# netneurolab/pypyls

Hardware: AMD Instinct MI355X
Metric: resamples/sec (perm+boot), behavioral_pls X(500x200000)/Y(500x50) fp64 (higher is better)
Workload: dtype f64

## Files before the change

pypyls_amd/csrc/plsx_compact.hip:

```cpp
#include "plsx_internal.h"

using namespace plsxi;

namespace plsxi {

template <int MT, int KT, bool TAIL = false>
int launch_xprod_cboot(plsx_ctx* ctx, int nres, int nks_c, SplitEpi se, hipStream_t st)
{
    const size_t stage = (size_t)2 * (((size_t)KT * MT * 64 + 127) / 128) * 128 * 8 + (size_t)nks_c * 4 * sizeof(int);
    const size_t epi = (size_t)se.npairs * 128 * 8 + (size_t)2 * MT * 16 * 4;
    const size_t lds = std::max(stage, epi);
    HIPCHK(set_lds(k_xprod_compact<MT, KT, 3, TAIL>, lds));
    const int ncolblk = ceil_div(ctx->Bpad, 128);
    KTimer tm(ctx, KC_XPROD, st);
    hipLaunchKernelGGL((k_xprod_compact<MT, KT, 3, TAIL>), dim3(round_up(ncolblk, 8) * round_up(nres, 8)), dim3(256),
                       lds, st, ptr<double>(ctx->Afrag_c), (size_t)nks_c * MT * 64, ptr<double>(ctx->Xc), ctx->Bpad, nks_c,
                       ptr<double>(ctx->R), ctx->Bpad, ctx->Tpp, ptr<int>(ctx->out_row_c), ptr<int>(ctx->mom_idx_c),
                       (const double*)nullptr, nres, ncolblk, se);
    LAUNCHCHK();
    return 0;
}

int launch_cboot(plsx_ctx* ctx, int nres, int nks_c, SplitEpi se, hipStream_t st)
{
    const int MTc = ceil_div(ctx->Tp, 16);
    const bool tail = ctx->Tp - (MTc - 1) * 16 <= 4 && MTc >= 2;
    switch (MTc) {
        case 1: return launch_xprod_cboot<1, 12>(ctx, nres, nks_c, se, st);
        case 2: return tail ? launch_xprod_cboot<2, 6, true>(ctx, nres, nks_c, se, st)
                            : launch_xprod_cboot<2, 6>(ctx, nres, nks_c, se, st);
        case 3: return tail ? launch_xprod_cboot<3, 4, true>(ctx, nres, nks_c, se, st)
                            : launch_xprod_cboot<3, 4>(ctx, nres, nks_c, se, st);
        case 4: return tail ? launch_xprod_cboot<4, PLSX_CKT, true>(ctx, nres, nks_c, se, st)
                            : launch_xprod_cboot<4, PLSX_CKT>(ctx, nres, nks_c, se, st);
#define PLSX_CB(M, K) case M: return tail ? launch_xprod_cboot<M, K, true>(ctx, nres, nks_c, se, st) \
                                          : launch_xprod_cboot<M, K>(ctx, nres, nks_c, se, st);
        PLSX_CB(5, 2) PLSX_CB(6, 2) PLSX_CB(7, 1) PLSX_CB(8, 1) PLSX_CB(9, 1) PLSX_CB(10, 1) PLSX_CB(11, 1) PLSX_CB(12, 1) PLSX_CB(13, 1)
#undef PLSX_CB
        default: return fail(ctx, PLSX_ERR_STATE, "compact bootstrap blocks: T' > 208");
    }
}
template <int MT, int KT, bool TAIL = false, int EPI = 5>
int launch_xprod_compact(plsx_ctx* ctx, int m, int nks_c, SplitEpi se, hipStream_t st)
{
    const int J = ctx->J;
    const size_t stage = (size_t)2 * (((size_t)KT * MT * 64 + 127) / 128) * 128 * 8 + (size_t)nks_c * 4 * sizeof(int);
    const size_t epi = EPI == 8 ? (size_t)MT * 16 * 4 : (size_t)5 * J * 128 * 8 + (size_t)2 * MT * 16 * 4 + (size_t)MT * 16 * 5 * 8;
    const size_t lds = std::max(stage, epi);
    se.off_pre = 0;
    HIPCHK(set_lds(k_xprod_compact<MT, KT, EPI, TAIL>, lds));
    const int ncolblk = ceil_div(ctx->Bpad, 128);
    KTimer tm(ctx, KC_XPROD, st);
    hipLaunchKernelGGL((k_xprod_compact<MT, KT, EPI, TAIL>), dim3(round_up(ncolblk, 8) * round_up(m, 8)), dim3(256), lds, st,
                       ptr<double>(ctx->Afrag_c), (size_t)nks_c * MT * 64, ptr<double>(ctx->Xc), ctx->Bpad, nks_c,
                       ptr<double>(ctx->R), ctx->Bpad, (EPI == 8 ? 1 : 2) * ctx->Tpp, ptr<int>(ctx->out_row_c), ptr<int>(ctx->mom_idx_c),
                       ptr<double>(ctx->momn_m), m, ncolblk, se);
    LAUNCHCHK();
    return 0;
}

int launch_csplit(plsx_ctx* ctx, int m, int nks_c, SplitEpi se, hipStream_t st, bool raw)
{
    const int MTc = ceil_div(ctx->Tp, 16);
    const bool tail = ctx->Tp - (MTc - 1) * 16 <= 4;
    if (raw) {
        switch (MTc) {
            case 2: return tail ? launch_xprod_compact<2, 6, true, 8>(ctx, m, nks_c, se, st)
                                : launch_xprod_compact<2, 6, false, 8>(ctx, m, nks_c, se, st);
            case 3: return tail ? launch_xprod_compact<3, 4, true, 8>(ctx, m, nks_c, se, st)
                                : launch_xprod_compact<3, 4, false, 8>(ctx, m, nks_c, se, st);
            case 4: if (tail) return launch_xprod_compact<4, PLSX_CKT, true, 8>(ctx, m, nks_c, se, st);
                    [[fallthrough]];
            default: return fail(ctx, PLSX_ERR_STATE, "raw compact split blocks: T' outside 17..52");
        }
    }
    switch (MTc) {
        case 1: return launch_xprod_compact<1, 12>(ctx, m, nks_c, se, st);
        case 2: return tail ? launch_xprod_compact<2, 6, true>(ctx, m, nks_c, se, st)
                            : launch_xprod_compact<2, 6>(ctx, m, nks_c, se, st);
        case 3: return tail ? launch_xprod_compact<3, 4, true>(ctx, m, nks_c, se, st)
                            : launch_xprod_compact<3, 4>(ctx, m, nks_c, se, st);
        default: return tail ? launch_xprod_compact<4, PLSX_CKT, true>(ctx, m, nks_c, se, st)
                             : launch_xprod_compact<4, PLSX_CKT>(ctx, m, nks_c, se, st);
    }
}

}
```

pypyls_amd/csrc/plsx_k_xprod.h:

```cpp
#pragma once
#include <type_traits>
#include <utility>

template <class F, int... I>
__device__ __forceinline__ void xprod_static_for(F&& f, std::integer_sequence<int, I...>)
{
    (f(std::integral_constant<int, I>()), ...);
}
#include "plsx_common.h"
#include "plsx_k_prep.h"

#define PLSX_RSRC_FLAGS 0x00020000
template <int NT, int PASSES, bool EVEN, int STAGE>
__device__ __forceinline__ void stage_copy_buf(const double* src, double* dst, int tid, int wave)
{
    __amdgpu_buffer_rsrc_t rs = __builtin_amdgcn_make_buffer_rsrc((void*)src, (short)0, 0x7fffffff,
                                                                   PLSX_RSRC_FLAGS);
    const int voff = tid * 16;
#pragma unroll
    for (int p = 0; p < PASSES; ++p) {
        if (EVEN || p * NT + wave * 64 < STAGE / 2) {
            __builtin_amdgcn_raw_ptr_buffer_load_lds(
                rs, (__attribute__((address_space(3))) void*)(dst + (size_t)(p * NT + wave * 64) * 2),
                16, voff, p * NT * 16, 0, 0);
        }
    }
}

__device__ __forceinline__ double load_x_buf(const double* rowbase, int voff)
{
    __amdgpu_buffer_rsrc_t rs = __builtin_amdgcn_make_buffer_rsrc((void*)rowbase, (short)0, 0x7fffffff,
                                                                   PLSX_RSRC_FLAGS);
    return __builtin_bit_cast(double, __builtin_amdgcn_raw_buffer_load_b64(rs, voff, 0, 0));
}

#define PLSX_ACC_PITCH 80
template <int MT, int NW, int KT, int NSQ, int EPI = 0>
__global__ __launch_bounds__(NW * 64, 2)
void k_xprod(const double* __restrict__ Afrag, size_t group_stride,
             const double* __restrict__ X, int ldx, int nks,
             double* __restrict__ R, int ldr, int rows_per_group,
             const int* __restrict__ out_row, const int* __restrict__ mom_idx,
             const double* __restrict__ mom_n, int nmom_pad,
             int n_groups, int ncolblk, double* __restrict__ mom_out, SplitEpi se, int ntab)
{
    extern __shared__ __attribute__((aligned(16))) double smem[];
    constexpr int NT = NW * 64;
    constexpr int STAGE = KT * MT * 64;
    constexpr int STAGE_LDS = ((STAGE + 127) / 128) * 128;
    constexpr int PASSES = (STAGE + NT * 2 - 1) / (NT * 2);
    constexpr bool EVEN = (STAGE % (NT * 2)) == 0;
    const int tid = threadIdx.x;
    const int lane = tid & 63, wave = tid >> 6;
    const int sweep = blockIdx.x / (8 * ncolblk);
    const int within = blockIdx.x - sweep * (8 * ncolblk);
    int grp = sweep * 8 + (within & 7);
    int colblk = within >> 3;
    if (sweep * 8 + 8 > n_groups) {
        const int rem = n_groups - sweep * 8;
        const int cnt = (rem * ncolblk + 7) >> 3;
        const int id = (within & 7) * cnt + colblk;
        if (colblk >= cnt || id >= rem * ncolblk) return;
        grp = sweep * 8 + id / ncolblk;
        colblk = id - (id / ncolblk) * ncolblk;
    }
    const int col = colblk * (NW * 16) + wave * 16 + (lane & 15);
    const int kq = lane >> 4;

    static_assert(EPI != 7 || KT == 1 || KT == 2 || KT == 4, "EPI 7: the four k-steps of a tile row are whole stages");
    const int qblk = (EPI == 7) ? grp / max(se.J, 1) : 0;
    const int ks0 = (EPI == 7) ? qblk * (MT * 4) : 0;
    if (EPI == 7) { X += (size_t)ks0 * 4 * ldx; nks -= ks0; }
    const double* Ag = Afrag + (size_t)grp * group_stride + (size_t)ks0 * (MT * 64);
    const int swave = __builtin_amdgcn_readfirstlane(wave);
    const int xvoff = (kq * ldx + min(col, ldx - 1)) * 8;

    d4 acc[MT];
#pragma unroll
    for (int m = 0; m < MT; ++m) acc[m] = (d4){0.0, 0.0, 0.0, 0.0};

    const int nkt = nks / KT;
    constexpr bool SPLIT = (EPI == 1);
    if constexpr (SPLIT) {
        if (se.off_pre > 0 && NW == 4) {
            double* sRf = smem + se.off_pre;
            double* sRc = sRf + se.Tpp * (NW * 16);
            __amdgpu_buffer_rsrc_t rsF = __builtin_amdgcn_make_buffer_rsrc(
                (void*)(se.Rfull + (size_t)colblk * (NW * 16)), (short)0, 0x7fffffff, PLSX_RSRC_FLAGS);
            const int vo = ((lane >> 5) * ldr + (lane & 31) * 2) * 8;
            for (int j = swave; j < se.Tpp / 2; j += NW)
                __builtin_amdgcn_raw_ptr_buffer_load_lds(
                    rsF, (__attribute__((address_space(3))) void*)(sRf + j * 128), 16, vo, j * 2 * ldr * 8, 0, 0);
            __amdgpu_buffer_rsrc_t rsC = __builtin_amdgcn_make_buffer_rsrc(
                (void*)(se.rowc + (size_t)grp * MT * 16 * 5), (short)0, 0x7fffffff, PLSX_RSRC_FLAGS);
            for (int pc = swave; pc < (MT * 16 * 5 + 127) / 128; pc += NW)
                __builtin_amdgcn_raw_ptr_buffer_load_lds(
                    rsC, (__attribute__((address_space(3))) void*)(sRc + pc * 128), 16, lane * 16, pc * 1024, 0, 0);
        }
    }
    stage_copy_buf<NT, PASSES, EVEN, STAGE>(Ag, smem, tid, swave);
    double xb[KT];
#pragma unroll
    for (int s = 0; s < KT; ++s)
        xb[s] = load_x_buf(X + (size_t)(s * 4) * ldx, xvoff);
#pragma unroll
    for (int s = 0; s < KT; ++s) asm volatile("" : "+v"(xb[s]));
    __syncthreads();

    auto pass = [&](int kt, auto na) {
        constexpr int NA = decltype(na)::value;
        const int cur = kt & 1;
        const int kn = min(kt + 1, nkt - 1);
        double xn[KT];
        stage_copy_buf<NT, PASSES, EVEN, STAGE>(Ag + (size_t)kn * STAGE, smem + (cur ^ 1) * STAGE_LDS, tid, swave);
#pragma unroll
        for (int s = 0; s < KT; ++s)
            xn[s] = load_x_buf(X + (size_t)((kn * KT + s) * 4) * ldx, xvoff);
        const double* sA = smem + cur * STAGE_LDS + lane;
#pragma unroll
        for (int s = 0; s < KT; ++s) {
            const double b = xb[s];
            const double bsq = (NSQ > 0) ? b * b : 0.0;
#pragma unroll
            for (int m = 0; m < NA; ++m)
                acc[m] = mfma_f64(sA[(s * MT + m) * 64], (m < MT - NSQ) ? b : bsq, acc[m]);
        }
#pragma unroll
        for (int s = 0; s < KT; ++s) xb[s] = xn[s];
        __syncthreads();
    };
    int kt_first = 0;
    if constexpr (EPI == 7) {
        xprod_static_for([&](auto mm) {
#pragma unroll
            for (int j = 0; j < 4 / KT; ++j) {
                const int kt = (4 / KT) * decltype(mm)::value + j;
                if (kt < nkt) pass(kt, std::integral_constant<int, decltype(mm)::value + 1>());
            }
        }, std::make_integer_sequence<int, MT>());
        kt_first = min(nkt, 4 * MT / KT);
    }
    for (int kt = kt_first; kt < nkt; ++kt) pass(kt, std::integral_constant<int, MT>());

    constexpr int W0 = MT - 2 * NSQ, SQ0 = MT - NSQ, NMOM = NSQ * 16;
    if constexpr (EPI == 6) {
        static_assert(MT == 2 * NSQ, "EPI 6 is a moment-only instantiation");
#pragma unroll
        for (int j = 0; j < NSQ; ++j)
#pragma unroll
            for (int i = 0; i < 4; ++i) {
                const int pair = grp * (NSQ * 16) + j * 16 + kq + 4 * i;
                if (pair >= se.npairs || col >= ldr) continue;
                se.scale[(size_t)pair * ldr + col] = acc[j][i];
                se.scale2[(size_t)pair * ldr + col] = acc[NSQ + j][i];
            }
        return;
    }
    if constexpr (EPI == 4) {
        static_assert(MT == 2 * NSQ, "EPI 4 is the moment-only instantiation");
#pragma unroll
        for (int j = 0; j < NSQ; ++j)
#pragma unroll
            for (int i = 0; i < 4; ++i) {
                const int pair = grp * (NSQ * 16) + j * 16 + kq + 4 * i;
                if (pair >= se.npairs || col >= ldr) continue;
                const double m1 = acc[j][i], m2 = acc[NSQ + j][i];
                const double nn = mom_n[pair];
                const double var = (m2 - m1 * m1 / nn) / (nn - 1.0);
                se.scale[(size_t)pair * ldr + col] = (var > 0.0) ? sd_rsqrt(var) : 0.0;
            }
        return;
    }
    if constexpr (EPI == 3) {
        const int nmu = se.npairs;
        double* sS3 = smem;
        int* s_out = reinterpret_cast<int*>(smem + (size_t)nmu * (NW * 16));
        int* s_mom = s_out + MT * 16;
        const double* sc0 = se.scale + (size_t)grp * nmu * ldr + colblk * (NW * 16);
        for (int idx = tid; idx < nmu * (NW * 16); idx += NT) {
            const int mi = idx / (NW * 16), c = idx - mi * (NW * 16);
            sS3[idx] = sc0[(size_t)mi * ldr + c];
        }
        for (int i = tid; i < MT * 16; i += NT) { s_out[i] = out_row[i]; s_mom[i] = mom_idx[i]; }
        __syncthreads();
        double* Rg = R + (size_t)grp * rows_per_group * ldr + col;
        const int cw = wave * 16 + (lane & 15);
        const int rows_valid = min(rows_per_group, se.accB - grp * rows_per_group);
#pragma unroll
        for (int m = 0; m < MT; ++m) {
            int orow[4];
            double sc[4];
#pragma unroll
            for (int i = 0; i < 4; ++i) {
                const int row = m * 16 + kq + 4 * i;
                orow[i] = s_out[row];
                const int mi = s_mom[row];
                sc[i] = mi >= 0 ? sS3[mi * (NW * 16) + cw] : 1.0;
            }
#pragma unroll
            for (int i = 0; i < 4; ++i)
                if (orow[i] >= 0 && orow[i] < rows_valid) Rg[(size_t)orow[i] * ldr] = acc[m][i] * sc[i];
        }
        return;
    }
    if constexpr (EPI == 7) {
        if (NW > 4 && col >= ldr) return;
        const int s0 = qblk * (MT * 16);
        const int Srows = se.accB;
        const double* Xc = X + col - (size_t)(ks0 * 4) * ldx;
        double part = 0.0;
#pragma unroll
        for (int m = 0; m < MT; ++m) {
            double xv[4];
#pragma unroll
            for (int i = 0; i < 4; ++i) {
                const int sr = s0 + m * 16 + kq + 4 * i;
                const double x = Xc[(size_t)min(sr, Srows - 1) * ldx];
                xv[i] = sr < Srows ? x : 0.0;
            }
#pragma unroll
            for (int i = 0; i < 4; ++i) part = __builtin_fma(xv[i], acc[m][i], part);
            asm volatile("" : "+v"(part));
        }
        part += __shfl_xor(part, 16);
        part += __shfl_xor(part, 32);
        if (kq == 0) se.acc_sum[(size_t)grp * ldr + col] = part;
        return;
    }
    if constexpr (EPI == 2) {
        constexpr int ACCP = NW * 16 + 16;
        constexpr int BCW = NW * 16;
        const int L = se.accL;
        double* sU = smem;
        double* sV = smem + (size_t)L * ACCP;
        double* sT = sV + (size_t)L * ACCP;
        int* s_l = reinterpret_cast<int*>(sT + 32 * ACCP);
        for (int i = tid; i < 2 * L * ACCP; i += NT) smem[i] = 0.0;
        for (int i = tid; i < MT * 16; i += NT) s_l[i] = out_row[i];
        const int cw = wave * 16 + (lane & 15);
#pragma unroll
        for (int m0 = 0; m0 < MT; m0 += 2) {
            __syncthreads();
#pragma unroll
            for (int mm = 0; mm < 2; ++mm)
#pragma unroll
                for (int i = 0; i < 4; ++i)
                    if (m0 + mm < MT) sT[(mm * 16 + kq + 4 * i) * ACCP + cw] = acc[m0 + mm][i];
            __syncthreads();
            for (int idx = tid; idx < L * BCW; idx += NT) {
                const int l = idx / BCW, c = idx - l * BCW;
                double u = sU[l * ACCP + c], v2 = sV[l * ACCP + c];
                for (int rl = 0; rl < 32 && m0 * 16 + rl < MT * 16; ++rl)
                    if (s_l[m0 * 16 + rl] == l) { const double v = sT[rl * ACCP + c]; u += v; v2 += v * v; }
                sU[l * ACCP + c] = u; sV[l * ACCP + c] = v2;
            }
        }
        __syncthreads();
        const int b0 = colblk * (NW * 16);
        double* ps = se.acc_sum + (size_t)grp * se.accB * L;
        double* pq = se.acc_sq + (size_t)grp * se.accB * L;
        for (int idx = tid; idx < NW * 16 * L; idx += NT) {
            const int c = idx / L, l = idx - c * L;
            if (b0 + c < se.accB) {
                ps[(size_t)(b0 + c) * L + l] = sU[l * ACCP + c];
                pq[(size_t)(b0 + c) * L + l] = sV[l * ACCP + c];
            }
        }
        return;
    }
    if constexpr (SPLIT && NSQ > 0) {
        const int nmu = se.nmu;
        const bool pre = se.off_pre > 0 && NW == 4;
        double* w5 = smem + wave * (5 * nmu * 16);
        int* s_out = reinterpret_cast<int*>(smem + NW * 5 * nmu * 16);
        int* s_mom = s_out + MT * 16;
        const double* sRf = smem + se.off_pre;
        double* s_rc = pre ? smem + se.off_pre + se.Tpp * (NW * 16)
                           : reinterpret_cast<double*>(s_mom + MT * 16);
        const int pitch2 = 2 * se.Tpp;
        for (int i = tid; i < MT * 16; i += NT) {
            const int orw = out_row[i];
            s_out[i] = orw < 0 ? -1 : (orw | ((orw % pitch2) << 20));
            s_mom[i] = mom_idx[i];
        }
        if (!pre)
            for (int i = tid; i < MT * 16 * 5; i += NT) s_rc[i] = se.rowc[(size_t)grp * MT * 16 * 5 + i];
#pragma unroll
        for (int j = 0; j < NSQ; ++j)
#pragma unroll
            for (int i = 0; i < 4; ++i) {
                const int mr = j * 16 + kq + 4 * i;
                if (mr >= nmu) continue;
                const int o = mr * 16 + (lane & 15);
                const double n1 = mom_n[(size_t)grp * nmom_pad + mr];
                const double m1 = acc[W0 + j][i], m2 = acc[SQ0 + j][i];
                const int jc = mr % se.J;
                const double nF = (double)se.cell_len[jc];
                const double SF = se.cellS1[(size_t)jc * ldr + col], SFF = se.cellS2[(size_t)jc * ldr + col];
                const double n2 = nF - n1;
                const bool ok = n1 > 1.5 && n2 > 1.5;
                const double var1 = ok ? (m2 - m1 * m1 / n1) / (n1 - 1.0) : 0.0;
                const double s2x = SF - m1, s2xx = SFF - m2;
                const double var2 = ok ? (s2xx - s2x * s2x / n2) / (n2 - 1.0) : 0.0;
                const double varF = (SFF - SF * SF / nF) / (nF - 1.0);
                w5[0 * nmu * 16 + o] = ok ? m1 / n1 : 0.0;
                w5[1 * nmu * 16 + o] = (var1 > 0.0) ? 1.0 / sqrt(var1) : 0.0;
                w5[2 * nmu * 16 + o] = ok ? s2x / n2 : 0.0;
                w5[3 * nmu * 16 + o] = (var2 > 0.0) ? 1.0 / sqrt(var2) : 0.0;
                w5[4 * nmu * 16 + o] = (varF > 0.0) ? sqrt(varF) : 0.0;
            }
        __syncthreads();
        double* Rg = R + (size_t)grp * rows_per_group * ldr + col;
#pragma unroll
        for (int m = 0; m < W0; ++m)
#pragma unroll
            for (int i = 0; i < 4; ++i) {
                const int row = m * 16 + kq + 4 * i;
                const int packed = s_out[row];
                if (packed < 0) continue;
                const int orow = packed & 0xfffff, t = packed >> 20;
                const int o = s_mom[row] * 16 + (lane & 15);
                const double* rc = s_rc + row * 5;
                const double c1 = acc[m][i];
                const double rf = pre ? sRf[t * (NW * 16) + wave * 16 + (lane & 15)]
                                      : se.Rfull[(size_t)t * ldr + col];
                const double cf = rf * rc[4] * w5[4 * nmu * 16 + o];
                const double r1 = (c1 - rc[0] * w5[o]) * rc[1] * w5[1 * nmu * 16 + o];
                const double r2 = ((cf - c1) - rc[2] * w5[2 * nmu * 16 + o]) * rc[3] * w5[3 * nmu * 16 + o];
                __builtin_nontemporal_store(r1, &Rg[(size_t)orow * ldr]);
                __builtin_nontemporal_store(r2, &Rg[(size_t)(orow + se.Tpp) * ldr]);
            }
        return;
    }
    double* sS = smem + wave * (2 * NMOM * 16);
    double* sQ = sS + NMOM * 16;
    int* s_out = reinterpret_cast<int*>(smem + NW * 2 * NMOM * 16);
    int* s_mom = s_out + MT * 16;
    const int tab = (ntab > 1) ? (grp % ntab) * (MT * 16) : 0;
    for (int i = tid; i < MT * 16; i += NT) { s_out[i] = out_row[tab + i]; s_mom[i] = mom_idx[tab + i]; }
    if (NSQ > 0) {
#pragma unroll
        for (int j = 0; j < NSQ; ++j)
#pragma unroll
            for (int i = 0; i < 4; ++i) {
                sS[j * 256 + (kq + 4 * i) * 16 + (lane & 15)] = acc[W0 + j][i];
                sQ[j * 256 + (kq + 4 * i) * 16 + (lane & 15)] = acc[SQ0 + j][i];
            }
    }
    __syncthreads();
    if (NSQ > 0) {
        for (int mr = kq; mr < NMOM; mr += 4) {
            const int o = mr * 16 + (lane & 15);
            const double m1 = sS[o], m2 = sQ[o];
            const double nn = mom_n[(size_t)grp * nmom_pad + mr];
            const double var = (m2 - m1 * m1 / nn) / (nn - 1.0);
            const double sc = (var > 0.0) ? 1.0 / sqrt(var) : 0.0;
            sS[o] = sc;
            if (mom_out) {
                double* mo = mom_out + ((size_t)grp * nmom_pad + mr) * 2 * ldr + col;
                mo[0] = m1 / nn;
                mo[ldr] = sc;
            }
        }
        __syncthreads();
    }
    if (NW > 4 && col >= ldr) return;
    double* Rg = R + (size_t)(ntab > 1 ? grp / ntab : grp) * rows_per_group * ldr + col;
#pragma unroll
    for (int m = 0; m < W0; ++m) {
        int orow[4];
        double sc[4];
#pragma unroll
        for (int i = 0; i < 4; ++i) {
            const int row = m * 16 + kq + 4 * i;
            orow[i] = s_out[row];
            const int mi = s_mom[row];
            sc[i] = (NSQ > 0 && mi >= 0) ? sS[mi * 16 + (lane & 15)] : 1.0;
        }
#pragma unroll
        for (int i = 0; i < 4; ++i)
            if (orow[i] >= 0) Rg[(size_t)orow[i] * ldr] = acc[m][i] * sc[i];
    }
}

__device__ __forceinline__ d2 load_x2_buf(const double* base, int voff)
{
    __amdgpu_buffer_rsrc_t rs = __builtin_amdgcn_make_buffer_rsrc((void*)base, (short)0, 0x7fffffff, PLSX_RSRC_FLAGS);
    return __builtin_bit_cast(d2, __builtin_amdgcn_raw_buffer_load_b128(rs, voff, 0, 0));
}

template <int MT, int KT, int EPI, bool TAIL>
__global__ __launch_bounds__(256, MT > 6 ? 2 : ((MT > 4 || (EPI == 5 && MT == 4 && !TAIL)) ? 3 : 4))
void k_xprod_compact(const double* __restrict__ Afrag, size_t group_stride,
                     const double* __restrict__ X, int ldx, int nks,
                     double* __restrict__ R, int ldr, int rows_per_group,
                     const int* __restrict__ out_row, const int* __restrict__ mom_idx,
                     const double* __restrict__ mom_n, int n_groups, int ncolblk, SplitEpi se)
{
    static_assert(EPI == 3 || EPI == 5 || EPI == 8, "compact blocks: bootstrap (3), fused split-half (5) or raw first-half sums (8)");
    extern __shared__ __attribute__((aligned(16))) double smem[];
    constexpr int NW = 4, NT = NW * 64, BC = NW * 32;
    constexpr int STAGE = KT * MT * 64;
    constexpr int STAGE_LDS = ((STAGE + 127) / 128) * 128;
    constexpr int PASSES = (STAGE + NT * 2 - 1) / (NT * 2);
    constexpr bool EVEN = (STAGE % (NT * 2)) == 0;
    constexpr int MF = TAIL ? MT - 1 : MT;
    const int tid = threadIdx.x, lane = tid & 63, wave = tid >> 6;
    const int ncb = (ncolblk + 7) & ~7;
    const int sweep = blockIdx.x / (8 * ncb);
    const int within = blockIdx.x - sweep * (8 * ncb);
    const int slot = within >> 3;
    const int grp = sweep * 8 + (slot & 7);
    const int colblk = (slot >> 3) * 8 + (within & 7);
    if (grp >= n_groups || colblk >= ncolblk) return;
    const int kq = lane >> 4;
    const int cw = wave * 32 + 2 * (lane & 15);
    const int col = colblk * BC + cw;
    const bool live = col < ldr;
    const int lcol = live ? col : 0;
    const double* Ag = Afrag + (size_t)grp * group_stride;
    const int swave = __builtin_amdgcn_readfirstlane(wave);

    d4 acc0[MF > 0 ? MF : 1], acc1[MF > 0 ? MF : 1];
#pragma unroll
    for (int m = 0; m < MF; ++m) { acc0[m] = (d4){0.0, 0.0, 0.0, 0.0}; acc1[m] = (d4){0.0, 0.0, 0.0, 0.0}; }
    double tl0 = 0.0, tl1 = 0.0;
    const int toff = (lane & 48) + (lane & 3) - lane;

    const int ksteps = max(1, (se.row_cnt[grp] + 3) >> 2);
    const int nkt = (ksteps + KT - 1) / KT;
    int* s_tab = reinterpret_cast<int*>(smem + 2 * STAGE_LDS);
    for (int i = tid; i < nks * 4; i += NT) s_tab[i] = se.row_tab[(size_t)grp * nks * 4 + i];
    __syncthreads();
    auto x_off = [&](int kstep) -> int { return (s_tab[kstep * 4 + kq] * ldx + lcol) * 8; };

    stage_copy_buf<NT, PASSES, EVEN, STAGE>(Ag, smem, tid, swave);
    d2 xb[KT];
#pragma unroll
    for (int s = 0; s < KT; ++s) xb[s] = load_x2_buf(X, x_off(s));
#pragma unroll
    for (int s = 0; s < KT; ++s) asm volatile("" : "+v"(xb[s]));
    __syncthreads();

    auto pass = [&](int kt, auto full) {
        const int cur = kt & 1;
        const int kn = min(kt + 1, nkt - 1);
        d2 xn[KT];
        stage_copy_buf<NT, PASSES, EVEN, STAGE>(Ag + (size_t)kn * STAGE, smem + (cur ^ 1) * STAGE_LDS, tid, swave);
#pragma unroll
        for (int s = 0; s < KT; ++s) xn[s] = load_x2_buf(X, x_off(kn * KT + s));
        const double* sA = smem + cur * STAGE_LDS + lane;
#pragma unroll
        for (int s = 0; s < KT; ++s) {
            if constexpr (!decltype(full)::value) {
                if (kt * KT + s >= ksteps) break;
            }
            const double b0 = xb[s].x, b1 = xb[s].y;
#pragma unroll
            for (int m = 0; m < MF; ++m) {
                const double a = sA[(s * MT + m) * 64];
                acc0[m] = mfma_f64(a, b0, acc0[m]);
                acc1[m] = mfma_f64(a, b1, acc1[m]);
            }
            if constexpr (TAIL) {
                const double a = sA[(s * MT + MT - 1) * 64 + toff];
                tl0 = mfma_f64_4x4(a, b0, tl0);
                tl1 = mfma_f64_4x4(a, b1, tl1);
            }
        }
#pragma unroll
        for (int s = 0; s < KT; ++s) xb[s] = xn[s];
        __syncthreads();
    };
    const int nfull = ksteps / KT;
    int kt_main = 0;
    for (; kt_main < nfull; ++kt_main) pass(kt_main, std::integral_constant<bool, true>());
    for (; kt_main < nkt; ++kt_main) pass(kt_main, std::integral_constant<bool, false>());

    auto val0 = [&](int m, int i) -> double { return (TAIL && m == MT - 1) ? tl0 : acc0[m < MF ? m : 0][i]; };
    auto val1 = [&](int m, int i) -> double { return (TAIL && m == MT - 1) ? tl1 : acc1[m < MF ? m : 0][i]; };

    if constexpr (EPI == 8) {
        int* s_out = reinterpret_cast<int*>(smem);
        for (int i = tid; i < MT * 16; i += NT) s_out[i] = out_row[i];
        __syncthreads();
        if (!live) return;
        double* Rg = R + (size_t)grp * rows_per_group * ldr + col;
#pragma unroll
        for (int m = 0; m < MT; ++m)
#pragma unroll
            for (int i = 0; i < 4; ++i) {
                if (TAIL && m == MT - 1 && i > 0) break;
                const int orow = s_out[m * 16 + kq + 4 * i];
                if (orow < 0) continue;
                __builtin_nontemporal_store((d2){val0(m, i), val1(m, i)}, reinterpret_cast<d2*>(&Rg[(size_t)orow * ldr]));
            }
        return;
    } else if constexpr (EPI == 3) {
        const int nmu = se.npairs;
        double* sS3 = smem;
        int* s_out = reinterpret_cast<int*>(smem + (size_t)nmu * BC);
        int* s_mom = s_out + MT * 16;
        const double* sc0 = se.scale + (size_t)grp * nmu * ldr + colblk * BC;
        for (int idx = tid; idx < nmu * BC; idx += NT) {
            const int mi = idx / BC, c = idx - mi * BC;
            sS3[idx] = (colblk * BC + c < ldr) ? sc0[(size_t)mi * ldr + c] : 0.0;
        }
        for (int i = tid; i < MT * 16; i += NT) { s_out[i] = out_row[i]; s_mom[i] = mom_idx[i]; }
        __syncthreads();
        if (!live) return;
        double* Rg = R + (size_t)grp * rows_per_group * ldr + col;
        const int rows_valid = min(rows_per_group, se.accB - grp * rows_per_group);
#pragma unroll
        for (int m = 0; m < MT; ++m)
#pragma unroll
            for (int i = 0; i < 4; ++i) {
                if (TAIL && m == MT - 1 && i > 0) break;
                const int row = m * 16 + kq + 4 * i;
                const int orow = s_out[row], mi = s_mom[row];
                if (orow < 0 || orow >= rows_valid) continue;
                d2 sc = (d2){1.0, 1.0};
                if (mi >= 0) sc = *reinterpret_cast<const d2*>(&sS3[mi * BC + cw]);
                *reinterpret_cast<d2*>(&Rg[(size_t)orow * ldr]) = (d2){val0(m, i) * sc.x, val1(m, i) * sc.y};
            }
        return;
    } else {
        const int J = se.J;
        double* w5 = smem;
        int* s_out = reinterpret_cast<int*>(smem + (size_t)5 * J * BC);
        int* s_mom = s_out + MT * 16;
        double* s_rc = reinterpret_cast<double*>(s_mom + MT * 16);
        const int pitch2 = 2 * se.Tpp;
        for (int i = tid; i < MT * 16; i += NT) {
            const int orw = out_row[i];
            s_out[i] = orw < 0 ? -1 : (orw | ((orw % pitch2) << 20));
            s_mom[i] = mom_idx[i];
        }
        for (int i = tid; i < MT * 16 * 5; i += NT) s_rc[i] = se.rowc[(size_t)grp * MT * 16 * 5 + i];
        const int cb0 = colblk * BC;
        for (int idx = tid; idx < J * BC; idx += NT) {
            const int jc = idx / BC, c = idx - jc * BC;
            double u1 = 0, v1 = 0, u2 = 0, v2 = 0, sF = 0;
            if (cb0 + c < ldr) {
                const size_t pair = (size_t)grp * J + jc;
                const double n1 = mom_n[pair];
                const double m1 = se.scale[pair * ldr + cb0 + c], m2 = se.scale2[pair * ldr + cb0 + c];
                const double nF = (double)se.cell_len[jc];
                const double SF = se.cellS1[(size_t)jc * ldr + cb0 + c], SFF = se.cellS2[(size_t)jc * ldr + cb0 + c];
                const double n2 = nF - n1;
                const bool ok = n1 > 1.5 && n2 > 1.5;
                const double var1 = ok ? (m2 - m1 * m1 / n1) / (n1 - 1.0) : 0.0;
                const double s2x = SF - m1, s2xx = SFF - m2;
                const double var2 = ok ? (s2xx - s2x * s2x / n2) / (n2 - 1.0) : 0.0;
                const double varF = (SFF - SF * SF / nF) / (nF - 1.0);
                u1 = ok ? m1 / n1 : 0.0;
                v1 = (var1 > 0.0) ? 1.0 / sqrt(var1) : 0.0;
                u2 = ok ? s2x / n2 : 0.0;
                v2 = (var2 > 0.0) ? 1.0 / sqrt(var2) : 0.0;
                sF = (varF > 0.0) ? sqrt(varF) : 0.0;
            }
            const int o = jc * BC + c;
            w5[0 * J * BC + o] = u1; w5[1 * J * BC + o] = v1; w5[2 * J * BC + o] = u2;
            w5[3 * J * BC + o] = v2; w5[4 * J * BC + o] = sF;
        }
        __syncthreads();
        if (!live) return;
        double* Rg = R + (size_t)grp * rows_per_group * ldr + col;
        const int JW = J * BC;
#pragma unroll
        for (int m = 0; m < MT; ++m)
#pragma unroll
            for (int i = 0; i < 4; ++i) {
                if (TAIL && m == MT - 1 && i > 0) break;
                const int row = m * 16 + kq + 4 * i;
                const int packed = s_out[row];
                if (packed < 0) continue;
                const int o = s_mom[row] * BC + cw;
                const double rc0 = s_rc[row * 5], rc1 = s_rc[row * 5 + 1];
                const d2 u1 = *reinterpret_cast<const d2*>(&w5[o]), v1 = *reinterpret_cast<const d2*>(&w5[JW + o]);
                const d2 r1 = (d2){(val0(m, i) - rc0 * u1.x) * rc1 * v1.x, (val1(m, i) - rc0 * u1.y) * rc1 * v1.y};
                __builtin_nontemporal_store(r1, reinterpret_cast<d2*>(&Rg[(size_t)(packed & 0xfffff) * ldr]));
            }
#pragma unroll
        for (int m0 = 0; m0 < MT; m0 += 2) {
            asm volatile("" ::: "memory");
            d2 rfv[2][4];
#pragma unroll
            for (int mm = 0; mm < 2; ++mm)
#pragma unroll
                for (int i = 0; i < 4; ++i) {
                    const int m = m0 + mm;
                    if (m >= MT || (TAIL && m == MT - 1 && i > 0)) break;
                    const int packed = s_out[m * 16 + kq + 4 * i];
                    rfv[mm][i] = packed < 0 ? (d2){0.0, 0.0}
                                            : *reinterpret_cast<const d2*>(&se.Rfull[(size_t)(packed >> 20) * ldr + col]);
                }
#pragma unroll
            for (int mm = 0; mm < 2; ++mm)
#pragma unroll
                for (int i = 0; i < 4; ++i) {
                    const int m = m0 + mm;
                    if (m >= MT || (TAIL && m == MT - 1 && i > 0)) break;
                    const int row = m * 16 + kq + 4 * i;
                    const int packed = s_out[row];
                    if (packed < 0) continue;
                    const int o = s_mom[row] * BC + cw;
                    const double rc2 = s_rc[row * 5 + 2], rc3 = s_rc[row * 5 + 3], rc4 = s_rc[row * 5 + 4];
                    const d2 u2 = *reinterpret_cast<const d2*>(&w5[2 * JW + o]), v2 = *reinterpret_cast<const d2*>(&w5[3 * JW + o]);
                    const d2 sF = *reinterpret_cast<const d2*>(&w5[4 * JW + o]);
                    const double c10 = val0(m, i), c11 = val1(m, i);
                    const double cf0 = rfv[mm][i].x * rc4 * sF.x, cf1 = rfv[mm][i].y * rc4 * sF.y;
                    const d2 r2 = (d2){((cf0 - c10) - rc2 * u2.x) * rc3 * v2.x, ((cf1 - c11) - rc2 * u2.y) * rc3 * v2.y};
                    __builtin_nontemporal_store(r2, reinterpret_cast<d2*>(&Rg[(size_t)((packed & 0xfffff) + se.Tpp) * ldr]));
                }
        }
    }
}
```

Measured before the change: 5956.

## Restructure compact xprod kernel prologue, double-buffer ping-pong and epilogue row maps

Reworks the compact cross-product kernel so the row-map and row-table staging overlaps with the first X and A loads. The table is pre-scaled by ldx*8, and the k-loop is unrolled into a static two-buffer ping-pong with register swap. In the bootstrap epilogue the output-row and moment-index maps are packed into one int. Scale factors come from registers when few pairs exist, otherwise they are loaded async to per-wave LDS. LDS sizing is centralised and occupancy hints per MT are retuned. The aim is fewer syncthreads, less epilogue staging and more occupancy, at the cost of added complexity and register pressure.

Result: faster. 6023, median of 6 (+1.1%).

```diff
diff --git a/pypyls_amd/csrc/plsx_compact.hip b/pypyls_amd/csrc/plsx_compact.hip
--- a/pypyls_amd/csrc/plsx_compact.hip
+++ b/pypyls_amd/csrc/plsx_compact.hip
@@ -7,9 +7,7 @@
 template <int MT, int KT, bool TAIL = false>
 int launch_xprod_cboot(plsx_ctx* ctx, int nres, int nks_c, SplitEpi se, hipStream_t st)
 {
-    const size_t stage = (size_t)2 * (((size_t)KT * MT * 64 + 127) / 128) * 128 * 8 + (size_t)nks_c * 4 * sizeof(int);
-    const size_t epi = (size_t)se.npairs * 128 * 8 + (size_t)2 * MT * 16 * 4;
-    const size_t lds = std::max(stage, epi);
+    const size_t lds = compact_lds_bytes(MT, KT, 3, nks_c, se.npairs);
     HIPCHK(set_lds(k_xprod_compact<MT, KT, 3, TAIL>, lds));
     const int ncolblk = ceil_div(ctx->Bpad, 128);
     KTimer tm(ctx, KC_XPROD, st);
@@ -44,9 +42,7 @@
 int launch_xprod_compact(plsx_ctx* ctx, int m, int nks_c, SplitEpi se, hipStream_t st)
 {
     const int J = ctx->J;
-    const size_t stage = (size_t)2 * (((size_t)KT * MT * 64 + 127) / 128) * 128 * 8 + (size_t)nks_c * 4 * sizeof(int);
-    const size_t epi = EPI == 8 ? (size_t)MT * 16 * 4 : (size_t)5 * J * 128 * 8 + (size_t)2 * MT * 16 * 4 + (size_t)MT * 16 * 5 * 8;
-    const size_t lds = std::max(stage, epi);
+    const size_t lds = compact_lds_bytes(MT, KT, EPI, nks_c, J);
     se.off_pre = 0;
     HIPCHK(set_lds(k_xprod_compact<MT, KT, EPI, TAIL>, lds));
     const int ncolblk = ceil_div(ctx->Bpad, 128);
diff --git a/pypyls_amd/csrc/plsx_k_xprod.h b/pypyls_amd/csrc/plsx_k_xprod.h
--- a/pypyls_amd/csrc/plsx_k_xprod.h
+++ b/pypyls_amd/csrc/plsx_k_xprod.h
@@ -389,8 +389,24 @@
     return __builtin_bit_cast(d2, __builtin_amdgcn_raw_buffer_load_b128(rs, voff, 0, 0));
 }
 
+__host__ __device__ constexpr int compact_stage_lds(int MT, int KT) { return ((KT * MT * 64 + 127) / 128) * 128; }
+__host__ __device__ constexpr int compact_scale_regs(int KT) { return KT < 4 ? KT : 4; }
+__host__ __device__ constexpr size_t compact_lds_bytes(int MT, int KT, int EPI, int nks, int J)
+{
+    const size_t loop = (size_t)MT * 16 * 8 + (size_t)2 * compact_stage_lds(MT, KT) * 8 + (size_t)nks * 4 * 4;
+    if (EPI == 3) return loop + (J > compact_scale_regs(KT) ? (size_t)J * 128 * 8 : 0);
+    const size_t epi5 = (size_t)MT * 16 * 8 + (size_t)5 * J * 128 * 8 + (size_t)MT * 16 * 5 * 8;
+    return EPI == 5 && epi5 > loop ? epi5 : loop;
+}
+
+__host__ __device__ constexpr int compact_waves(int MT, int EPI, bool TAIL)
+{
+    if (EPI == 3) return MT > 10 ? 2 : MT == 10 ? (TAIL ? 3 : 2) : MT > 6 ? 3 : MT > 4 ? 4 : (MT == 4 && TAIL) ? 5 : 4;
+    return (EPI == 5 && MT == 4 && !TAIL) ? 3 : 4;
+}
+
 template <int MT, int KT, int EPI, bool TAIL>
-__global__ __launch_bounds__(256, MT > 6 ? 2 : ((MT > 4 || (EPI == 5 && MT == 4 && !TAIL)) ? 3 : 4))
+__global__ __launch_bounds__(256, compact_waves(MT, EPI, TAIL))
 void k_xprod_compact(const double* __restrict__ Afrag, size_t group_stride,
                      const double* __restrict__ X, int ldx, int nks,
                      double* __restrict__ R, int ldr, int rows_per_group,
@@ -401,11 +417,12 @@
     extern __shared__ __attribute__((aligned(16))) double smem[];
     constexpr int NW = 4, NT = NW * 64, BC = NW * 32;
     constexpr int STAGE = KT * MT * 64;
-    constexpr int STAGE_LDS = ((STAGE + 127) / 128) * 128;
+    constexpr int STAGE_LDS = compact_stage_lds(MT, KT);
     constexpr int PASSES = (STAGE + NT * 2 - 1) / (NT * 2);
     constexpr bool EVEN = (STAGE % (NT * 2)) == 0;
     constexpr int MF = TAIL ? MT - 1 : MT;
-    const int tid = threadIdx.x, lane = tid & 63, wave = tid >> 6;
+    constexpr int NSCR = compact_scale_regs(KT);
+    static_assert(MT * 16 <= NT, "the row maps are staged by one thread per row");
     const int ncb = (ncolblk + 7) & ~7;
     const int sweep = blockIdx.x / (8 * ncb);
     const int within = blockIdx.x - sweep * (8 * ncb);
@@ -413,49 +430,87 @@
     const int grp = sweep * 8 + (slot & 7);
     const int colblk = (slot >> 3) * 8 + (within & 7);
     if (grp >= n_groups || colblk >= ncolblk) return;
+    const double* Ag = Afrag + (size_t)grp * group_stride;
+    const int swave = __builtin_amdgcn_readfirstlane((int)threadIdx.x >> 6);
+
+    d4 acc0[MF > 0 ? MF : 1], acc1[MF > 0 ? MF : 1];
+#pragma unroll
+    for (int m = 0; m < MF; ++m) { acc0[m] = (d4){0.0, 0.0, 0.0, 0.0}; acc1[m] = (d4){0.0, 0.0, 0.0, 0.0}; }
+    double tl0 = 0.0, tl1 = 0.0;
+
+    int* s_out = reinterpret_cast<int*>(smem);
+    int* s_mom = s_out + MT * 16;
+    double* sStage = smem + MT * 16;
+    int* s_tab = reinterpret_cast<int*>(sStage + 2 * STAGE_LDS);
+    const int J3 = se.npairs;
+    double* sW = reinterpret_cast<double*>(s_tab + nks * 4) + swave * (J3 * 32);
+    d2 scr[NSCR];
+    {
+    const int tid = threadIdx.x, lane = tid & 63, wave = tid >> 6;
     const int kq = lane >> 4;
     const int cw = wave * 32 + 2 * (lane & 15);
     const int col = colblk * BC + cw;
     const bool live = col < ldr;
-    const int lcol = live ? col : 0;
-    const double* Ag = Afrag + (size_t)grp * group_stride;
-    const int swave = __builtin_amdgcn_readfirstlane(wave);
-
-    d4 acc0[MF > 0 ? MF : 1], acc1[MF > 0 ? MF : 1];
-#pragma unroll
-    for (int m = 0; m < MF; ++m) { acc0[m] = (d4){0.0, 0.0, 0.0, 0.0}; acc1[m] = (d4){0.0, 0.0, 0.0, 0.0}; }
-    double tl0 = 0.0, tl1 = 0.0;
+    const int lcol8 = (live ? col : 0) * 8;
     const int toff = (lane & 48) + (lane & 3) - lane;
 
+    const int* tabg = se.row_tab + (size_t)grp * nks * 4;
+    const int ldx8 = ldx * 8;
+    int row0[KT];
+#pragma unroll
+    for (int s = 0; s < KT; ++s) row0[s] = tabg[s * 4 + kq];
+    stage_copy_buf<NT, PASSES, EVEN, STAGE>(Ag, sStage, tid, swave);
+    int orw = -1, mix = -1;
+    if (tid < MT * 16) {
+        orw = out_row[tid];
+        if (EPI != 8) mix = mom_idx[tid];
+    }
     const int ksteps = max(1, (se.row_cnt[grp] + 3) >> 2);
     const int nkt = (ksteps + KT - 1) / KT;
-    int* s_tab = reinterpret_cast<int*>(smem + 2 * STAGE_LDS);
-    for (int i = tid; i < nks * 4; i += NT) s_tab[i] = se.row_tab[(size_t)grp * nks * 4 + i];
+    const int ntab = nkt * KT * 4;
+    auto tab_load = [&](int i0, int (&v)[4]) {
+#pragma unroll
+        for (int u = 0; u < 4; ++u) v[u] = tabg[min(i0 + u * NT + tid, ntab - 1)];
+#pragma unroll
+        for (int u = 0; u < 4; ++u) asm volatile("" : "+v"(v[u]));
+    };
+    auto tab_store = [&](int i0, const int (&v)[4]) {
+#pragma unroll
+        for (int u = 0; u < 4; ++u)
+            if (i0 + u * NT + tid < ntab) s_tab[i0 + u * NT + tid] = v[u] * ldx8;
+    };
+    int tv[4];
+    tab_load(0, tv);
+    d2 xa[KT], xb[KT];
+#pragma unroll
+    for (int s = 0; s < KT; ++s) xa[s] = load_x2_buf(X, row0[s] * ldx8 + lcol8);
+    tab_store(0, tv);
+    for (int i0 = 4 * NT; i0 < ntab; i0 += 4 * NT) { tab_load(i0, tv); tab_store(i0, tv); }
+    if (tid < MT * 16) {
+        if constexpr (EPI == 3) {
+            const int rows_valid = min(rows_per_group, se.accB - grp * rows_per_group);
+            s_out[tid] = (orw < 0 || orw >= rows_valid) ? -1 : (orw | ((mix + 1) << 16));
+        } else if constexpr (EPI == 5) {
+            s_out[tid] = orw < 0 ? -1 : (orw | ((orw % (2 * se.Tpp)) << 20));
+            s_mom[tid] = mix;
+        } else {
+            s_out[tid] = orw;
+        }
+    }
+#pragma unroll
+    for (int s = 0; s < KT; ++s) asm volatile("" : "+v"(xa[s]));
     __syncthreads();
-    auto x_off = [&](int kstep) -> int { return (s_tab[kstep * 4 + kq] * ldx + lcol) * 8; };
-
-    stage_copy_buf<NT, PASSES, EVEN, STAGE>(Ag, smem, tid, swave);
-    d2 xb[KT];
-#pragma unroll
-    for (int s = 0; s < KT; ++s) xb[s] = load_x2_buf(X, x_off(s));
-#pragma unroll
-    for (int s = 0; s < KT; ++s) asm volatile("" : "+v"(xb[s]));
-    __syncthreads();
-
-    auto pass = [&](int kt, auto full) {
-        const int cur = kt & 1;
-        const int kn = min(kt + 1, nkt - 1);
-        d2 xn[KT];
-        stage_copy_buf<NT, PASSES, EVEN, STAGE>(Ag + (size_t)kn * STAGE, smem + (cur ^ 1) * STAGE_LDS, tid, swave);
-#pragma unroll
-        for (int s = 0; s < KT; ++s) xn[s] = load_x2_buf(X, x_off(kn * KT + s));
-        const double* sA = smem + cur * STAGE_LDS + lane;
+
+    const double* sA0 = sStage + lane;
+    const double* sT0 = sA0 + toff;
+    auto contract = [&](auto curc, const d2 (&xc)[KT], auto full, int nlive) {
+        const int cur = curc;
+        const double* sA = sA0 + cur * STAGE_LDS;
+        const double* sT = sT0 + cur * STAGE_LDS;
 #pragma unroll
         for (int s = 0; s < KT; ++s) {
-            if constexpr (!decltype(full)::value) {
-                if (kt * KT + s >= ksteps) break;
-            }
-            const double b0 = xb[s].x, b1 = xb[s].y;
+            if (!decltype(full)::value && s >= nlive) continue;
+            const double b0 = xc[s].x, b1 = xc[s].y;
 #pragma unroll
             for (int m = 0; m < MF; ++m) {
                 const double a = sA[(s * MT + m) * 64];
@@ -463,27 +518,70 @@
                 acc1[m] = mfma_f64(a, b1, acc1[m]);
             }
             if constexpr (TAIL) {
-                const double a = sA[(s * MT + MT - 1) * 64 + toff];
+                const double a = sT[(s * MT + MT - 1) * 64];
                 tl0 = mfma_f64_4x4(a, b0, tl0);
                 tl1 = mfma_f64_4x4(a, b1, tl1);
             }
         }
-#pragma unroll
-        for (int s = 0; s < KT; ++s) xb[s] = xn[s];
+    };
+    const int* tp = s_tab + KT * 4 + kq;
+    const double* An = Ag + STAGE;
+    auto pass = [&](auto curc, const d2 (&xc)[KT], d2 (&xn)[KT]) {
+        constexpr int CUR = decltype(curc)::value;
+        stage_copy_buf<NT, PASSES, EVEN, STAGE>(An, sStage + (CUR ^ 1) * STAGE_LDS, tid, swave);
+#pragma unroll
+        for (int s = 0; s < KT; ++s) xn[s] = load_x2_buf(X, tp[s * 4] + lcol8);
+        An += STAGE;
+        tp += KT * 4;
+        contract(curc, xc, std::true_type(), KT);
         __syncthreads();
     };
-    const int nfull = ksteps / KT;
-    int kt_main = 0;
-    for (; kt_main < nfull; ++kt_main) pass(kt_main, std::integral_constant<bool, true>());
-    for (; kt_main < nkt; ++kt_main) pass(kt_main, std::integral_constant<bool, false>());
-
+    auto last = [&](int cur, const d2 (&xc)[KT]) {
+#pragma unroll
+        for (int j = 0; j < NSCR; ++j) scr[j] = (d2){1.0, 1.0};
+        if constexpr (EPI == 3) {
+            if (J3 <= NSCR) {
+#pragma unroll
+                for (int j = 0; j < NSCR; ++j)
+                    if (j < J3)
+                        scr[j] = *reinterpret_cast<const d2*>(
+                            reinterpret_cast<const char*>(se.scale + ((size_t)grp * J3 + j) * ldr) + lcol8);
+            } else if (live) {
+                __amdgpu_buffer_rsrc_t rs = __builtin_amdgcn_make_buffer_rsrc(
+                    (void*)(se.scale + (size_t)grp * J3 * ldr + colblk * BC + swave * 32), (short)0, 0x7fffffff, PLSX_RSRC_FLAGS);
+                const int ln4 = __lane_id() * 4;
+                for (int j = 0; j < J3; ++j)
+                    __builtin_amdgcn_raw_ptr_buffer_load_lds(
+                        rs, (__attribute__((address_space(3))) void*)(sW + j * 32), 4, ln4, j * ldr * 8, 0, 0);
+            }
+        }
+        contract(cur, xc, std::false_type(), ksteps - (nkt - 1) * KT);
+        if constexpr (EPI == 5) __syncthreads();
+    };
+    {
+        std::integral_constant<int, 0> c0;
+        std::integral_constant<int, 1> c1;
+        int kt = 0, cur = 0;
+        for (; kt + 2 < nkt; kt += 2) { pass(c0, xa, xb); pass(c1, xb, xa); }
+        if (kt + 1 < nkt) {
+            pass(c0, xa, xb);
+#pragma unroll
+            for (int s = 0; s < KT; ++s) xa[s] = xb[s];
+            cur = 1;
+        }
+        last(cur, xa);
+    }
+    }
+
+    int tid16 = threadIdx.x * 16;
+    if constexpr (EPI != 5) asm volatile("" : "+v"(tid16));
+    const int tid = tid16 >> 4, lane = tid & 63, wave = tid >> 6, kq = lane >> 4;
+    const int cw = wave * 32 + 2 * (lane & 15), col = colblk * BC + cw;
+    const bool live = col < ldr;
     auto val0 = [&](int m, int i) -> double { return (TAIL && m == MT - 1) ? tl0 : acc0[m < MF ? m : 0][i]; };
     auto val1 = [&](int m, int i) -> double { return (TAIL && m == MT - 1) ? tl1 : acc1[m < MF ? m : 0][i]; };
 
     if constexpr (EPI == 8) {
-        int* s_out = reinterpret_cast<int*>(smem);
-        for (int i = tid; i < MT * 16; i += NT) s_out[i] = out_row[i];
-        __syncthreads();
         if (!live) return;
         double* Rg = R + (size_t)grp * rows_per_group * ldr + col;
 #pragma unroll
@@ -497,45 +595,32 @@
             }
         return;
     } else if constexpr (EPI == 3) {
-        const int nmu = se.npairs;
-        double* sS3 = smem;
-        int* s_out = reinterpret_cast<int*>(smem + (size_t)nmu * BC);
-        int* s_mom = s_out + MT * 16;
-        const double* sc0 = se.scale + (size_t)grp * nmu * ldr + colblk * BC;
-        for (int idx = tid; idx < nmu * BC; idx += NT) {
-            const int mi = idx / BC, c = idx - mi * BC;
-            sS3[idx] = (colblk * BC + c < ldr) ? sc0[(size_t)mi * ldr + c] : 0.0;
-        }
-        for (int i = tid; i < MT * 16; i += NT) { s_out[i] = out_row[i]; s_mom[i] = mom_idx[i]; }
-        __syncthreads();
         if (!live) return;
+        if (J3 > NSCR) asm volatile("s_waitcnt vmcnt(0)" ::: "memory");
         double* Rg = R + (size_t)grp * rows_per_group * ldr + col;
-        const int rows_valid = min(rows_per_group, se.accB - grp * rows_per_group);
 #pragma unroll
         for (int m = 0; m < MT; ++m)
 #pragma unroll
             for (int i = 0; i < 4; ++i) {
                 if (TAIL && m == MT - 1 && i > 0) break;
-                const int row = m * 16 + kq + 4 * i;
-                const int orow = s_out[row], mi = s_mom[row];
-                if (orow < 0 || orow >= rows_valid) continue;
+                const int packed = s_out[m * 16 + kq + 4 * i];
+                if (packed < 0) continue;
+                const int orow = packed & 0xffff, mi = (packed >> 16) - 1;
                 d2 sc = (d2){1.0, 1.0};
-                if (mi >= 0) sc = *reinterpret_cast<const d2*>(&sS3[mi * BC + cw]);
+                if (J3 > NSCR) {
+                    if (mi >= 0) sc = *reinterpret_cast<const d2*>(&sW[mi * 32 + 2 * (lane & 15)]);
+                } else {
+#pragma unroll
+                    for (int j = 0; j < NSCR; ++j)
+                        if (mi == j) sc = scr[j];
+                }
                 *reinterpret_cast<d2*>(&Rg[(size_t)orow * ldr]) = (d2){val0(m, i) * sc.x, val1(m, i) * sc.y};
             }
         return;
     } else {
         const int J = se.J;
-        double* w5 = smem;
-        int* s_out = reinterpret_cast<int*>(smem + (size_t)5 * J * BC);
-        int* s_mom = s_out + MT * 16;
-        double* s_rc = reinterpret_cast<double*>(s_mom + MT * 16);
-        const int pitch2 = 2 * se.Tpp;
-        for (int i = tid; i < MT * 16; i += NT) {
-            const int orw = out_row[i];
-            s_out[i] = orw < 0 ? -1 : (orw | ((orw % pitch2) << 20));
-            s_mom[i] = mom_idx[i];
-        }
+        double* w5 = sStage;
+        double* s_rc = w5 + (size_t)5 * J * BC;
         for (int i = tid; i < MT * 16 * 5; i += NT) s_rc[i] = se.rowc[(size_t)grp * MT * 16 * 5 + i];
         const int cb0 = colblk * BC;
         for (int idx = tid; idx < J * BC; idx += NT) {
```
